# for-the-juan/SpGEMM

Hardware: AMD Instinct MI355X
Metric: SpGEMM GFLOPS (fp64, C=A^2) + achieved HBM GB/s fraction, 1/2/4/8 MI355X (higher is better)
Workload: dtype f64

## Files before the change

spgemm_amd/csrc/tsg_rows.hip:

```cpp
#include "tsg_internal.h"
#include "tsg_dev_common.h"

#include <cstdio>
#include <cstdlib>

namespace tsg {

namespace {

constexpr int S16_MAX = 16;
constexpr int RS_MAX = 64;
constexpr int CP_CH = 2048;
constexpr int S16_U = 2, S64_U = 2;
constexpr int M0_CAP = 256, M0_RUNS = 62, M0_NT = 64;
constexpr int M1_CAP = 512, M1_RUNS = 124, M1_NT = 128;
constexpr int M2_CAP = 1024, M2_RUNS = 248, M2_NT = 256;
constexpr int M3_CAP = 2048, M3_RUNS = 504, M3_NT = 512;
constexpr int M4_CAP = 4096, M4_RUNS = 512, M4_NT = 1024;
constexpr int W_CH = 32768;
constexpr int NCLS = 8;
constexpr int DR_SMAX = 4096;
constexpr int DR_CH = 16384;
constexpr int DR_GR = 16;
constexpr int DR_GMAX = 8192;
// ... 174 lines not shown
    if (P <= RS_MAX && k <= RS_MAX) return 1;
    if (P <= M0_CAP && k <= M0_RUNS) return 2;
    if (P <= M1_CAP && k <= M1_RUNS) return 3;
    if (P <= M2_CAP && k <= M2_RUNS) return 4;
    if (P <= M3_CAP && k <= M3_RUNS) return 5;
    if (P <= M4_CAP && k <= M4_RUNS) return 6;
    return 7;
}

__global__ __launch_bounds__(WG) void k_rows_bin(const int *rpA, int m, const long long *E, const long long *Etot,
                                                 int *rnnz, int4 *lists, int *cls, long long *soff,
                                                 unsigned long long *hst, const int *spart, int snb, int *sflag) {
    __shared__ int gb[NCLS];
    __shared__ long long red64[WAVES];
    constexpr int RPT = BIN_ROWS / WG;
    __shared__ int wcu[RPT][NCLS][WAVES];
    const int tid = threadIdx.x, lane = lane_id(), wv = wave_id();
    const int r0 = blockIdx.x * BIN_ROWS, r1 = min(m, r0 + BIN_ROWS);
    if (blockIdx.x == 0 && tid == 0) {
        hst[2] = (unsigned long long)*Etot;
        rnnz[m] = 0;
    }
    if (blockIdx.x == 0 && spart) {
        long long v = 0;
#pragma unroll 8
        for (int i = tid; i < snb; i += WG) v += spart[i];
        v = block_sum(v, red64);
        if (tid == 0 && v != 0) __hip_atomic_store(sflag, 1, __ATOMIC_RELAXED, __HIP_MEMORY_SCOPE_SYSTEM);
    }
    long long hp = 0, pmax = 0, drp = 0, hubr = 0, hbig = 0;
    int cu[RPT];
    int ra0[RPT], ra1[RPT];
#pragma unroll
    for (int u = 0; u < RPT; ++u) {
        const int r = r0 + u * WG + tid;
        ra0[u] = r < r1 ? rpA[r] : 0;
        ra1[u] = r < r1 ? rpA[r + 1] : 0;
    }
    long long e0[RPT], e1[RPT];
#pragma unroll
    for (int u = 0; u < RPT; ++u) {
        e0[u] = E[ra0[u]];
        e1[u] = E[ra1[u]];
    }
#pragma unroll
    for (int u = 0; u < RPT; ++u) {
        const int r = r0 + u * WG + tid;
        cu[u] = -1;
        if (r >= r1) continue;
        const long long P = e1[u] - e0[u];
        const int c = row_class(P, ra1[u] - ra0[u]);
        soff[r] = e0[u];
        cu[u] = c;
        if (c < 0) rnnz[r] = 0;
        hp += c == NCLS - 1 ? P : 0;
        hbig += c == NCLS - 1 && P <= kRowsHubProducts && P > OW_CH ? P - OW_CH : 0;
        pmax = max(pmax, P);
        if (P > kRowsHubProducts) drp += P;
        if (c == NCLS - 1 && ra1[u] - ra0[u] > OW_RUNS) ++hubr;
    }
    hp = block_sum(hp, red64);
    drp = block_sum(drp, red64);
    hubr = block_sum(hubr, red64);
    hbig = block_sum(hbig, red64);
#pragma unroll
    for (int d = 32; d > 0; d >>= 1) pmax = max(pmax, __shfl_xor(pmax, d, 64));
    if (lane == 0) red64[wv] = pmax;
    __syncthreads();
    if (tid == 0) {
        for (int w = 1; w < WAVES; ++w) pmax = max(pmax, red64[w]);
        if (hp) atomicAdd(&hst[0], (unsigned long long)hp);
        if (pmax) atomicMax(&hst[1], (unsigned long long)pmax);
        if (drp) atomicAdd(&hst[3], (unsigned long long)drp);
        if (hubr) atomicAdd(&hst[4], (unsigned long long)hubr);
        if (hbig) atomicAdd(&hst[8], (unsigned long long)hbig);
    }
    u64 mine[RPT];
#pragma unroll
    for (int u = 0; u < RPT; ++u) {
        mine[u] = 0;
#pragma unroll
        for (int t = 0; t < NCLS; ++t) {
            const u64 bt = __ballot(cu[u] == t);
            if (cu[u] == t) mine[u] = bt;
            if (lane == 0) wcu[u][t][wv] = __popcll(bt);
        }
    }
    __syncthreads();
    if (tid < NCLS) {
        int run = 0;
        for (int u = 0; u < RPT; ++u)
            for (int w = 0; w < WAVES; ++w) {
                const int v = wcu[u][tid][w];
                wcu[u][tid][w] = run;
                run += v;
            }
        gb[tid] = run ? atomicAdd(&cls[tid], run) : 0;
    }
    __syncthreads();
#pragma unroll
    for (int u = 0; u < RPT; ++u) {
        const int c = cu[u];
        if (c >= 0) {
            const int r = r0 + u * WG + tid;
            lists[(long)c * m + gb[c] + wcu[u][c][wv] + lanes_below(mine[u])] = make_int4(r, ra0[u], ra1[u] - ra0[u], 0);
        }
    }
}

constexpr int OH_NT = 1024, OH_PER = 8, OH_MAX = OH_NT * OH_PER, OH_NB = 64;
__global__ __launch_bounds__(OH_NT) void k_rows_order_h(const long long *E, const int *cls, int4 *list) {
    __shared__ int cnt[OH_NB];
    const int tid = threadIdx.x;
    const int n = cls[NCLS - 1];
    if (n < 2 || n > OH_MAX) return;
    if (tid < OH_NB) cnt[tid] = 0;
    __syncthreads();
    int4 r[OH_PER];
    int b[OH_PER];
#pragma unroll
    for (int u = 0; u < OH_PER; ++u) {
        const int i = u * OH_NT + tid;
        r[u] = i < n ? list[i] : make_int4(-1, 0, 0, 0);
    }
#pragma unroll
    for (int u = 0; u < OH_PER; ++u)
        if (r[u].x >= 0) {
            const long long P = E[r[u].y + r[u].z] - E[r[u].y];
            b[u] = OH_NB - 1 - (int)min((long long)OH_NB - 1, P >> 10);
            atomicAdd(&cnt[b[u]], 1);
        }
    __syncthreads();
    if (tid < 64) {
        const int v = cnt[tid];
        const int inc = wave_incl_scan_dpp(v);
        cnt[tid] = inc - v;
    }
    __syncthreads();
#pragma unroll
    for (int u = 0; u < OH_PER; ++u)
        if (r[u].x >= 0) list[atomicAdd(&cnt[b[u]], 1)] = r[u];
}

template <int J> __device__ __forceinline__ int row_bcast16(int v) {
    return __builtin_amdgcn_update_dpp(0, v, 0x150 | J, 0xf, 0xf, false);
}
template <int V> struct IntC { static constexpr int value = V; };
template <int J, int N, class F> __device__ __forceinline__ void static_for(F &&f) {
    if constexpr (J < N) {
        f(IntC<J>{});
        static_for<J + 1, N>(f);
    }
}

template <int G, int U>
__global__ __launch_bounds__(WG) void k_rows_small(RowsArgs g) {
    constexpr int RPW = 64 / G;
    __shared__ u64 sk[WAVES][U][64];
    __shared__ double sv[WAVES][U][64];
    const int lane = lane_id(), wv = wave_id(), sl = lane % G, gb = lane - sl;
    const int w0 = (blockIdx.x * WAVES + wv) * RPW * U;
    if (w0 >= g.nrows) return;
    int r[U], a0[U], k[U];
    bool live[U];
    long long base[U];
#pragma unroll
    for (int u = 0; u < U; ++u) {
        const int i = w0 + u * RPW + lane / G;
        live[u] = i < g.nrows;
        r[u] = 0, a0[u] = 0, k[u] = 0;
        if (live[u]) {
            const int4 e = g.list[i];
            r[u] = e.x;
            a0[u] = e.y;
            k[u] = e.z;
        }
    }
    int2 be[U];
    double av[U];
#pragma unroll
    for (int u = 0; u < U; ++u) {
        be[u] = make_int2(0, 0);
        av[u] = 0.0;
        base[u] = 0;
        if (live[u]) base[u] = g.E[a0[u]];
        if (sl < k[u]) {
            be[u] = g.ebnd[a0[u] + sl];
            av[u] = g.vA[a0[u] + sl];
        }
    }
    int P[U], pp[U];
    double ra[U];
#pragma unroll
    for (int u = 0; u < U; ++u) {
        const int len = be[u].y - be[u].x, bs = be[u].x;
        int inc = len;
        inc += dpp_mov<0x111, 0xf>(0, inc);
        inc += dpp_mov<0x112, 0xf>(0, inc);
        inc += dpp_mov<0x114, 0xf>(0, inc);
        inc += dpp_mov<0x118, 0xf>(0, inc);
        if constexpr (G == 64) {
            inc += dpp_mov<0x142, 0xa>(0, inc);
            inc += dpp_mov<0x143, 0xc>(0, inc);
        }
        const int roff = sl < k[u] ? inc - len : INT_MAX;
        int run = 0;
        if constexpr (G == 64) {
            P[u] = __shfl(inc, G - 1, G);
            for (int j = 1; j < k[u]; ++j) run = (__builtin_amdgcn_readlane(roff, j) <= sl) ? j : run;
        } else {
            static_assert(G == 16, "row broadcasts: 16-lane groups");
            P[u] = row_bcast16<15>(inc);
            static_for<1, 16>([&](auto jc) {
                constexpr int j = decltype(jc)::value;
                run = row_bcast16<j>(roff) <= sl ? j : run;
            });
        }
        const int rs = __shfl(roff, run, G), rb = __shfl(bs, run, G);
        ra[u] = __shfl(av[u], run, G);
        pp[u] = rb + sl - rs;
    }
    u64 key[U];
    double x[U];
#pragma unroll
    for (int u = 0; u < U; ++u) {
        key[u] = ~0ull;
        x[u] = 0.0;
        if (sl < P[u]) {
            key[u] = ((u64)(u32)g.Bcol[pp[u]] << 32) | (u32)sl;
            x[u] = g.Bval[pp[u]];
        }
    }
#pragma unroll
    for (int u = 0; u < U; ++u) {
        const u32 khi = (u32)(key[u] >> 32), klo = (u32)key[u];
        int rank = 0;
        if constexpr (G == 64) {
            for (int f = 0; f < P[u]; ++f) {
                const u64 kf = ((u64)(u32)__builtin_amdgcn_readlane((int)khi, f) << 32) |
                               (u32)__builtin_amdgcn_readlane((int)klo, f);
                rank += kf < key[u];
            }
        } else {
            const u64 ku = key[u];
            static_for<0, 16>([&](auto fc) {
                constexpr int f = decltype(fc)::value;
                const u64 kf = ((u64)(u32)row_bcast16<f>((int)khi) << 32) | (u32)row_bcast16<f>((int)klo);
                rank += kf < ku;
            });
        }
        if (sl < P[u]) {
            sk[wv][u][gb + rank] = key[u];
            sv[wv][u][gb + rank] = ra[u] * x[u];
        }
    }
    wave_lds_sync();
    const u64 gm = (G == 64 ? ~0ull : ((1ull << (G & 63)) - 1ull)) << gb;
#pragma unroll
    for (int u = 0; u < U; ++u) {
        int col = -1;
        bool head = false;
        if (sl < P[u]) {
            col = key_col(sk[wv][u][gb + sl]);
            head = sl == 0 || key_col(sk[wv][u][gb + sl - 1]) != col;
        }
        const u64 hb = __ballot(head) & gm;
        if (head) {
            double sm = sv[wv][u][gb + sl];
            for (int j = sl + 1; j < P[u] && key_col(sk[wv][u][gb + j]) == col; ++j) sm += sv[wv][u][gb + j];
            const long long o = base[u] + (long long)lanes_below(hb);
            g.Scol[o] = col;
            g.Sval[o] = sm;
        }
        if (live[u] && sl == 0) g.rnnz[r[u]] = __popcll(hb);
    }
}

template <int U, class T>
__device__ __forceinline__ void search_ilp(const T *a, int (&b)[U], int (&len)[U], const T (&key)[U],
                                           const bool (&ub)[U]) {
    for (;;) {
        bool more = false;
#pragma unroll
        for (int u = 0; u < U; ++u) more |= len[u] > 0;
        if (!more) break;
#pragma unroll
        for (int u = 0; u < U; ++u) {
            const int half = len[u] >> 1, idx = b[u] + half;
            const T v = a[len[u] > 0 ? idx : 0];
            const bool go = len[u] > 0 && (v < key[u] || (ub[u] && v == key[u]));
            b[u] = go ? idx + 1 : b[u];
            len[u] = go ? len[u] - half - 1 : half;
        }
    }
}

template <int D> __device__ __forceinline__ u32 lane_xor(u32 v) {
    if constexpr (D == 1) return (u32)__builtin_amdgcn_mov_dpp((int)v, 0xB1, 0xf, 0xf, false);
    else if constexpr (D == 2) return (u32)__builtin_amdgcn_mov_dpp((int)v, 0x4E, 0xf, 0xf, false);
    else if constexpr (D < 32) return (u32)__builtin_amdgcn_ds_swizzle((int)v, (D << 10) | 0x1f);
    else return (u32)__shfl_xor((int)v, D, 64);
}

template <int K, int J> __device__ __forceinline__ void bitonic_stage(u32 (&x)[4], int lane) {
    if constexpr (J >= 4) {
        constexpr int D = J / 4;
        const bool asc = K >= 256 || (lane & (K / 4)) == 0;
        const bool keep_max = asc != ((lane & D) == 0);
#pragma unroll
        for (int u = 0; u < 4; ++u) {
            const u32 y = lane_xor<D>(x[u]);
            x[u] = ((y < x[u]) != keep_max) ? y : x[u];
        }
    } else {
#pragma unroll
        for (int u = 0; u < 4; ++u)
            if ((u & J) == 0) {
                if constexpr (K < 4 || K >= 256) {
                    const bool asc = K < 4 ? (u & K) == 0 : true;
                    const u32 lo = min(x[u], x[u + J]), hi = max(x[u], x[u + J]);
                    x[u] = asc ? lo : hi;
                    x[u + J] = asc ? hi : lo;
                } else {
                    const bool desc = (lane & (K / 4)) != 0;
                    const bool sw = (x[u + J] < x[u]) != desc;
                    const u32 a = x[u], b = x[u + J];
                    x[u] = sw ? b : a;
                    x[u + J] = sw ? a : b;
                }
            }
    }
}
template <int K, int J> __device__ __forceinline__ void bitonic_merge(u32 (&x)[4], int lane) {
    bitonic_stage<K, J>(x, lane);
    if constexpr (J > 1) bitonic_merge<K, J / 2>(x, lane);
}
template <int K> __device__ __forceinline__ void bitonic_sort(u32 (&x)[4], int lane) {
    if constexpr (K > 2) bitonic_sort<K / 2>(x, lane);
    bitonic_merge<K, K / 2>(x, lane);
}
__device__ __forceinline__ void wave_sort256(u32 (&x)[4], int lane) { bitonic_sort<256>(x, lane); }

template <int NT, int CAP, int RUNS>
__global__ __launch_bounds__(NT, NT == 1024 ? 8 : 1) void k_rows_merge(RowsArgs g) {
    constexpr int NW = NT / 64;
    constexpr int IPM = (CAP + NT - 1) / NT | 1;
    constexpr int IB = CAP == 256 ? 8 : CAP == 512 ? 9 : CAP == 1024 ? 10 : CAP == 2048 ? 11 : 12;
    static_assert((1 << IB) == CAP, "CAP: a power of two in [256, 4096]");
    constexpr int SEG = 256;
    static_assert(CAP == 4 * NT, "four positions per thread");
    static_assert(RUNS <= NT, "a thread per A entry");
    __shared__ __align__(16) u32 kp[2][2][CAP];
    __shared__ int roff[RUNS + 1];
    __shared__ int rbs[RUNS];
    __shared__ double rav[RUNS];
    __shared__ int red[2 * NW];
    RP_INIT
    const int tid = threadIdx.x, lane = lane_id(), wv = wave_id();
    const int4 le = g.list[blockIdx.x];
    int2 be = make_int2(0, 0);
    double av = 0.0;
    if (tid < le.z) {
        be = g.ebnd[le.y + tid];
        av = g.vA[le.y + tid];
    }
    const long long base = g.E[le.y];
    double *const V = reinterpret_cast<double *>(kp[1][0]);
    {
        const int r = le.x;
        int k = 0, P = 0;
        {
            const int len = be.y - be.x;
            const u64 b = __ballot(len > 0);
            const int inc = wave_incl_scan_dpp(len);
            if (lane == 63) {
                red[wv] = __popcll(b);
                red[NW + wv] = inc;
            }
            __syncthreads();
            int off = 0, loff = 0;
#pragma unroll
            for (int w = 0; w < NW; ++w) {
                off += w < wv ? red[w] : 0;
                k += red[w];
                loff += w < wv ? red[NW + w] : 0;
                P += red[NW + w];
            }
            if (len > 0) {
                const int d = off + lanes_below(b);
                roff[d] = loff + inc - len;
                rbs[d] = be.x;
                rav[d] = av;
            }
            if (tid == 0) roff[k] = P;
            __syncthreads();
        }
        RP(0);
        const int e0 = wv * SEG + 4 * lane, ne = max(0, min(4, P - e0));
        int c[4] = {0, 0, 0, 0};
        u32 py[4] = {0, 0, 0, 0};
        double xv[4] = {0.0, 0.0, 0.0, 0.0};
        {
            int j = 0;
            if (ne > 0) j = lower_bound_dev(roff, 0, k + 1, e0 + 1) - 1;
            int pa[4] = {0, 0, 0, 0};
            double ra[4] = {0.0, 0.0, 0.0, 0.0}, bv[4] = {0.0, 0.0, 0.0, 0.0};
#pragma unroll
            for (int u = 0; u < 4; ++u)
                if (u < ne) {
                    const int q = e0 + u;
                    while (roff[j + 1] <= q) ++j;
                    pa[u] = rbs[j] + q - roff[j];
                    py[u] = ((u32)j << 16) | (u32)(q - roff[j]);
                    ra[u] = rav[j];
                }
#pragma unroll
            for (int u = 0; u < 4; ++u)
                if (u < ne) {
                    c[u] = g.Bcol[pa[u]];
                    bv[u] = g.Bval[pa[u]];
                }
#pragma unroll
            for (int u = 0; u < 4; ++u) xv[u] = u < ne ? ra[u] * bv[u] : 0.0;
        }
        int clo = INT_MAX, chi = -1;
#pragma unroll
        for (int u = 0; u < 4; ++u)
            if (u < ne) {
                clo = min(clo, c[u]);
                chi = max(chi, c[u]);
            }
        clo = wave_last(wave_incl_dpp(clo, INT_MAX, OpMin{}));
        chi = wave_last(wave_incl_dpp(chi, INT_MIN, OpMax{}));
        if (lane == 0) {
            red[wv] = clo;
            red[NW + wv] = chi;
        }
        __syncthreads();
        clo = red[0];
        chi = red[NW];
#pragma unroll
        for (int w = 1; w < NW; ++w) {
            clo = min(clo, red[w]);
            chi = max(chi, red[NW + w]);
        }
        const bool packed = (u32)(chi - clo) < (1u << (32 - IB)) - 1u;
        int npow = SEG;
        while (npow < P) npow <<= 1;
        u32 x[4] = {~0u, ~0u, ~0u, ~0u};
        if (packed) {
#pragma unroll
            for (int u = 0; u < 4; ++u) x[u] = u < ne ? ((u32)(c[u] - clo) << IB) | (u32)(e0 + u) : ~0u;
            if (ne > 0) {
                reinterpret_cast<double4 *>(V)[e0 >> 2] = make_double4(xv[0], xv[1], xv[2], xv[3]);
            }
            if (wv * SEG < P) wave_sort256(x, lane);
            if (wv * SEG < npow) *reinterpret_cast<uint4 *>(kp[0][0] + e0) = make_uint4(x[0], x[1], x[2], x[3]);
        } else {
#pragma unroll
            for (int u = 0; u < 4; ++u)
                if (u < ne) {
                    kp[0][0][e0 + u] = (u32)c[u];
                    kp[0][1][e0 + u] = py[u];
                }
        }
        __syncthreads();
        RP(1);
        int src = 0;
        if (packed) {
            const bool act = wv * SEG < npow;
            auto cmpx = [&](const uint4 y, bool rev, bool keep_min) {
                const u32 yy[4] = {rev ? y.w : y.x, rev ? y.z : y.y, rev ? y.y : y.z, rev ? y.x : y.w};
#pragma unroll
                for (int u = 0; u < 4; ++u) x[u] = keep_min ? min(x[u], yy[u]) : max(x[u], yy[u]);
            };
            for (int K = 2 * SEG; K <= npow; K <<= 1) {
                if (act) cmpx(*reinterpret_cast<const uint4 *>(kp[0][src] + (e0 ^ (K - 4))), true, (e0 & (K >> 1)) == 0);
                for (int J = K >> 2; J >= SEG; J >>= 1) {
                    src ^= 1;
                    if (act) *reinterpret_cast<uint4 *>(kp[0][src] + e0) = make_uint4(x[0], x[1], x[2], x[3]);
                    __syncthreads();
                    if (act) cmpx(*reinterpret_cast<const uint4 *>(kp[0][src] + (e0 ^ J)), false, (e0 & J) == 0);
                }
                if (act) bitonic_merge<256, 128>(x, lane);
                src ^= 1;
                if (act) *reinterpret_cast<uint4 *>(kp[0][src] + e0) = make_uint4(x[0], x[1], x[2], x[3]);
                __syncthreads();
            }
        }
        const int ipt = ((P + NT - 1) / NT) | 1;
        const int q0 = min(P, tid * ipt), q1 = min(P, q0 + ipt), nq = q1 - q0;
        if (!packed) {
            const int *const bd = roff;
            const int nb = k;
            int j0 = 0;
            if (nq > 0) j0 = lower_bound_dev(roff, 0, k + 1, q0 + 1) - 1;
            for (int lw = 0; (1 << lw) < nb; ++lw) {
                const u32 *ik = kp[src][0], *ip = kp[src][1];
                u32 *ok = kp[src ^ 1][0], *op = kp[src ^ 1][1];
                int pr = j0 >> (lw + 1);
                for (int q = q0; q < q1;) {
                    while (bd[min((pr + 1) << (lw + 1), nb)] <= q) ++pr;
                    const int ps = bd[pr << (lw + 1)];
                    const int pm = bd[min((2 * pr + 1) << lw, nb)];
                    const int pe = bd[min((pr + 1) << (lw + 1), nb)];
                    const int la = pm - ps, lb = pe - pm, qq = q - ps;
                    int lo = max(0, qq - lb), hi = min(qq, la);
                    while (lo < hi) {
                        const int t = (lo + hi) >> 1;
                        if (ik[ps + t] <= ik[pm + qq - t - 1]) lo = t + 1; else hi = t;
                    }
                    int ia = lo, ib = qq - lo;
                    u32 ka = ia < la ? ik[ps + ia] : ~0u, kbv = ib < lb ? ik[pm + ib] : ~0u;
                    const int qe = min(q1, pe);
                    for (; q < qe; ++q) {
                        const bool ta = ka <= kbv;
                        ok[q] = ta ? ka : kbv;
                        op[q] = ta ? ps + ia : pm + ib;
                        ia += ta;
                        ib += !ta;
                        const u32 kn = ik[ta ? ps + ia : pm + ib];
                        const bool live = ta ? ia < la : ib < lb;
                        ka = ta ? (live ? kn : ~0u) : ka;
                        kbv = ta ? kbv : (live ? kn : ~0u);
                    }
                }
#pragma unroll
                for (int u = 0; u < IPM; ++u)
                    if (u < nq) op[q0 + u] = ip[op[q0 + u]];
                __syncthreads();
                src ^= 1;
            }
        }
        RP(2);
        int nh = 0;
        const int np = packed ? max(0, min(4, P - e0)) : 0;
        double xs[4] = {0.0, 0.0, 0.0, 0.0};
        u32 hd = 0;
        const u32 *const sk = packed ? kp[0][src] : kp[src][0];
        double *const vb = reinterpret_cast<double *>(kp[src ^ 1][0]);
        if (packed) {
            const u32 prev = e0 > 0 && np > 0 ? sk[e0 - 1] : ~0u;
#pragma unroll
            for (int u = 0; u < 4; ++u)
                if (u < np) {
                    xs[u] = V[x[u] & (CAP - 1)];
                    const u32 pk = u ? x[u - 1] : prev;
                    hd |= (e0 + u == 0 || (x[u] >> IB) != (pk >> IB)) ? 1u << u : 0u;
                }
            nh = __popc(hd);
        } else {
            const u32 *sp = kp[src][1];
            int pa[IPM] = {};
            double ra[IPM] = {};
#pragma unroll
            for (int u = 0; u < IPM; ++u)
                if (u < nq) {
                    const u32 key = sk[q0 + u];
                    const u32 pj = sp[q0 + u];
                    const int ru = (int)(pj >> 16);
                    pa[u] = rbs[ru] + (int)(pj & 0xffffu);
                    ra[u] = rav[ru];
                    nh += (q0 + u == 0 || key != sk[q0 + u - 1]);
                }
            double xx[IPM] = {};
#pragma unroll
            for (int u = 0; u < IPM; ++u)
                if (u < nq) xx[u] = ra[u] * g.Bval[pa[u]];
#pragma unroll
            for (int u = 0; u < IPM; ++u)
                if (u < nq) vb[q0 + u] = xx[u];
        }
        const int inc = wave_incl_scan_dpp(nh);
        if (lane == 63) red[wv] = inc;
        __syncthreads();
        RP(3);
        int o = inc - nh, tot = 0;
#pragma unroll
        for (int w = 0; w < NW; ++w) {
            o += w < wv ? red[w] : 0;
            tot += red[w];
        }
        if (tid == 0) g.rnnz[r] = tot;
        if (packed) {
#pragma unroll
            for (int u = 0; u < 4; ++u)
                if (hd >> u & 1u) {
                    const u32 col = x[u] >> IB;
                    double sum = xs[u];
                    int j = u + 1;
#pragma unroll
                    for (int v = u + 1; v < 4; ++v)
                        if (j == v && v < np && (x[v] >> IB) == col) {
                            sum += xs[v];
                            ++j;
                        }
                    if (j == 4)
                        for (int q = e0 + 4; q < P && (sk[q] >> IB) == col; ++q) sum += V[sk[q] & (CAP - 1)];
                    g.Scol[base + o] = (int)col + clo;
                    g.Sval[base + o] = sum;
                    ++o;
                }
        } else {
            for (int q = q0; q < q1; ++q) {
                const u32 col = sk[q];
                if (q == 0 || sk[q - 1] != col) {
                    double sum = vb[q];
                    for (int j = q + 1; j < P && sk[j] == col; ++j) sum += vb[j];
                    g.Scol[base + o] = (int)col;
                    g.Sval[base + o] = sum;
                    ++o;
                }
            }
        }
        RP(4);
    }
    RP_DONE(CAP <= M1_CAP ? 2 : 1);
}

struct WalkTab {
    int pre[RH_NT];
    int bs[RH_NT];
    double av[RH_NT];
    int red[RH_NT / 64];
    int tot;
};
__device__ __forceinline__ void rows_batch(const RowsArgs &g, int a0, int k, int b0, WalkTab &tb) {
    constexpr int NW = RH_NT / 64;
    const int tid = threadIdx.x, lane = lane_id(), wv = wave_id();
    const int j = b0 + tid;
    int2 be = make_int2(0, 0);
    double av = 0.0;
    if (j < k) {
        be = g.ebnd[a0 + j];
        av = g.vA[a0 + j];
    }
    const int len = be.y - be.x;
    const int inc = wave_incl_scan_dpp(len);
    if (lane == 63) tb.red[wv] = inc;
    __syncthreads();
    int woff = 0, tot = 0;
#pragma unroll
    for (int w = 0; w < NW; ++w) {
        const int v = tb.red[w];
        woff += w < wv ? v : 0;
        tot += v;
    }
    tb.pre[tid] = woff + inc - len;
    tb.bs[tid] = be.x;
    tb.av[tid] = av;
    if (tid == 0) tb.tot = tot;
    __syncthreads();
}
__device__ __forceinline__ void batch_runmap(const WalkTab &tb, int nb, int qb, unsigned short *rmap, int *red) {
    constexpr int NW = RH_NT / 64;
    const int tid = threadIdx.x, lane = lane_id(), wv = wave_id();
    reinterpret_cast<uint2 *>(rmap)[tid] = make_uint2(0u, 0u);
    __syncthreads();
    if (tid < nb) {
        const int p0 = tb.pre[tid], p1 = tid + 1 < nb ? tb.pre[tid + 1] : tb.tot;
        if (p1 > p0 && p1 > qb && p0 < qb + 4 * RH_NT) rmap[max(p0, qb) - qb] = (unsigned short)tid;
    }
    __syncthreads();
    uint2 v = reinterpret_cast<const uint2 *>(rmap)[tid];
    int m[4];
    m[0] = (int)(v.x & 0xffffu);
    m[1] = max(m[0], (int)(v.x >> 16));
    m[2] = max(m[1], (int)(v.y & 0xffffu));
    m[3] = max(m[2], (int)(v.y >> 16));
    const int inc = wave_incl_dpp(m[3], 0, OpMax{});
    if (lane == 63) red[wv] = inc;
    int carry = __shfl_up(inc, 1, 64);
    if (lane == 0) carry = 0;
    __syncthreads();
#pragma unroll
    for (int w = 0; w < NW; ++w) carry = w < wv ? max(carry, red[w]) : carry;
    v.x = (u32)max(m[0], carry) | ((u32)max(m[1], carry) << 16);
    v.y = (u32)max(m[2], carry) | ((u32)max(m[3], carry) << 16);
    reinterpret_cast<uint2 *>(rmap)[tid] = v;
    __syncthreads();
}

template <bool VAL, class F>
__device__ __forceinline__ void batch_walk(const RowsArgs &g, int nb, int q0, int q1, const WalkTab &tb, F &&f,
                                           unsigned short *rmap, int *red) {
    constexpr int U = 4;
    const int tid = threadIdx.x;
    if (q0 >= q1) return;
    int c[U], cn[U];
    double x[U], xn[U];
    auto fetch = [&](int qb, unsigned short *rm, int (&cc)[U], double (&xx)[U]) {
        __syncthreads();
        batch_runmap(tb, nb, qb, rm, red);
#pragma unroll
        for (int u = 0; u < U; ++u) {
            const int q = qb + u * RH_NT + tid;
            const int r = q < q1 ? rm[u * RH_NT + tid] : 0;
            const int bs = tb.bs[r], pre = tb.pre[r];
            const int pp = q < q1 ? bs + q - pre : 0;
            cc[u] = g.Bcol[pp];
            if (VAL) xx[u] = g.Bval[pp];
        }
    };
    auto use = [&](int qb, const unsigned short *rm, const int (&cc)[U], const double (&xx)[U]) {
#pragma unroll
        for (int u = 0; u < U; ++u) {
            const bool ok = qb + u * RH_NT + tid < q1;
            f(cc[u], VAL && ok ? tb.av[rm[u * RH_NT + tid]] * xx[u] : 0.0, ok);
        }
    };
    constexpr int STEP = U * RH_NT;
    unsigned short *const rm0 = rmap, *const rm1 = rmap + 4 * RH_NT;
    fetch(q0, rm0, c, x);
#pragma unroll
    for (int st = 0; st < W_CH / STEP; st += 2) {
        const int qb = q0 + st * STEP;
        if (qb >= q1) break;
        fetch(qb + STEP, rm1, cn, xn);
        use(qb, rm0, c, x);
        if (qb + STEP >= q1) break;
        fetch(qb + 2 * STEP, rm0, c, x);
        use(qb + STEP, rm1, cn, xn);
    }
}

__device__ __forceinline__ int bm_rank(const u64 *bm, const u16 *g4, const int *blk, long long c) {
    const int w = (int)(c >> 6), gi = w >> 2, sub = w & 3;
    const ulonglong2 lo = reinterpret_cast<const ulonglong2 *>(bm)[gi * 2];
    const ulonglong2 hi = reinterpret_cast<const ulonglong2 *>(bm)[gi * 2 + 1];
    const u64 word = sub == 0 ? lo.x : sub == 1 ? lo.y : sub == 2 ? hi.x : hi.y;
    int rk = blk[w / RH_BLK] + g4[gi] + __popcll(word & ((1ull << (c & 63)) - 1ull));
    rk += sub > 0 ? __popcll(lo.x) : 0;
    rk += sub > 1 ? __popcll(lo.y) : 0;
    rk += sub > 2 ? __popcll(hi.x) : 0;
    return rk;
}

__global__ __launch_bounds__(RH_NT) void k_rows_bitmap(RowsArgs g, int *Tc, double *Tx, int *Tr,
                                                      unsigned long long *tcur) {
    {
        const int4 le0 = g.list[blockIdx.x];
        if (g.E[le0.y + le0.z] - g.E[le0.y] > kRowsHubProducts) return;
    }
    __shared__ __align__(16) u64 bm[RH_WORDS];
    __shared__ u16 g4[RH_NGRP];
    __shared__ int blk[RH_NBLK];
    __shared__ WalkTab wt;
    __shared__ int red[3 * (RH_NT / 64)];
    constexpr int NW = RH_NT / 64;
    RP_INIT
    const int tid = threadIdx.x, lane = lane_id(), wv = wave_id();
    const int4 le = g.list[blockIdx.x];
    const int r = le.x, a0 = le.y, k = le.z;
    const long long base = g.E[a0];
    if (k > OW_RUNS) return;
    const int P = (int)(g.E[a0 + k] - base);
    int *const opre = reinterpret_cast<int *>(&wt);
    int *const obs = opre + OW_RUNS;
    int lo = INT_MAX, hi = -1;
    {
        int2 be0 = make_int2(0, 0), be1 = make_int2(0, 0);
        if (2 * tid < k) be0 = g.ebnd[a0 + 2 * tid];
        if (2 * tid + 1 < k) be1 = g.ebnd[a0 + 2 * tid + 1];
        const int l0 = be0.y - be0.x, l1 = be1.y - be1.x;
        const int f0 = l0 > 0 ? g.Bcol[be0.x] : INT_MAX, e0 = l0 > 0 ? g.Bcol[be0.y - 1] : -1;
        const int f1 = l1 > 0 ? g.Bcol[be1.x] : INT_MAX, e1 = l1 > 0 ? g.Bcol[be1.y - 1] : -1;
        const int inc = wave_incl_scan_dpp(l0 + l1);
        lo = wave_last(wave_incl_dpp(min(f0, f1), INT_MAX, OpMin{}));
        hi = wave_last(wave_incl_dpp(max(e0, e1), INT_MIN, OpMax{}));
        if (lane == 63) red[wv] = inc;
        if (lane == 0) {
            red[NW + wv] = lo;
            red[2 * NW + wv] = hi;
        }
        __syncthreads();
        int woff = 0;
#pragma unroll
        for (int w = 0; w < NW; ++w) {
            woff += w < wv ? red[w] : 0;
            lo = min(lo, red[NW + w]);
            hi = max(hi, red[2 * NW + w]);
        }
        const int ex = woff + inc - l0 - l1;
        opre[2 * tid] = ex;
        opre[2 * tid + 1] = ex + l0;
        obs[2 * tid] = be0.x;
        obs[2 * tid + 1] = be1.x;
    }
    if ((long long)hi - lo >= RH_SPAN) return;
    {
        __shared__ long long s_toff;
        if (tid == 0 && P > OW_CH) s_toff = (long long)atomicAdd(tcur, (unsigned long long)(P - OW_CH));
// ... 400 lines not shown
    for (int t = 0; t < PT; ++t) {
        const int w = tid * PT + t;
        v[t] = w < nw ? in[u0 + w] : 0;
        sum += v[t];
    }
    const int inc = wave_incl_scan_dpp(sum);
    if (lane == 63) red[wv] = inc;
    __syncthreads();
    int off = inc - sum, tot = 0;
#pragma unroll
    for (int w = 0; w < NW; ++w) {
        off += w < wv ? red[w] : 0;
        tot += red[w];
    }
    long long rb = 0;
    int lo = 0, wb = 0, row = 0;
    if (rec) {
        const int4 le = g.list[blockIdx.x];
        rb = g.E[le.y];
        row = le.x;
        lo = wlo[blockIdx.x];
        wb = wwb[blockIdx.x];
    }
#pragma unroll
    for (int t = 0; t < PT; ++t) {
        const int w = tid * PT + t;
        if (w < nw) {
            out[u0 + w] = off;
            if (rec) rec[u0 + w] = WUnit{rb + off, lo + (w << wb), wb, v[t], row};
        }
        off += v[t];
    }
    if (rnnz && tid == 0) rnnz[g.list[blockIdx.x].x] = tot;
    if (ulist) {
        constexpr int HEAVY = W_RPT * WU_NT;
        int ns = 0, nh = 0, nm = 0;
#pragma unroll
        for (int t = 0; t < PT; ++t) {
            ns += v[t] > 0 && v[t] <= WS_MAX;
            nh += v[t] > HEAVY;
            nm += v[t] > WS_MAX && v[t] <= HEAVY;
        }
        const int is = wave_incl_scan_dpp(ns), ih = wave_incl_scan_dpp(nh), im = wave_incl_scan_dpp(nm);
        unsigned long long old = 0;
        if (lane == 63 && (is | ih | im))
            old = atomicAdd(lcnt64, (unsigned long long)is | ((unsigned long long)ih << 21) |
                                        ((unsigned long long)im << 42));
        old = ((unsigned long long)__shfl((int)(old >> 32), 63, 64) << 32) | (u32)__shfl((int)old, 63, 64);
        int ps = (int)(old & 0x1fffff) + is - ns, ph = (int)((old >> 21) & 0x1fffff) + ih - nh,
            pm = (int)(old >> 42) + im - nm;
#pragma unroll
        for (int t = 0; t < PT; ++t) {
            const int w = tid * PT + t;
            if (v[t] > 0 && v[t] <= WS_MAX) ulist[ps++] = u0 + w;
            else if (v[t] > HEAVY) ulist2[nu - 1 - ph++] = u0 + w;
            else if (v[t] > WS_MAX) ulist2[pm++] = u0 + w;
        }
    }
}

__global__ __launch_bounds__(W_NT) __attribute__((amdgpu_waves_per_eu(8, 8))) void k_rows_wscatter(RowsArgs g, const int4 *chunks, const long long *cmoff,
                                                       const int *wlo, const int *wwb, const int *ubase,
                                                       const int *ubo, const int *cbo) {
    __shared__ __align__(16) unsigned char lds[W_MAXW * 4 + 8 * RH_NT * 2];
    __shared__ WalkTab wt;
    __shared__ int red[W_NT / 64];
    int *const cur = reinterpret_cast<int *>(lds);
    unsigned short *const rm = reinterpret_cast<unsigned short *>(lds + W_MAXW * 4);
    const int tid = threadIdx.x;
    const int4 ch = chunks[blockIdx.x];
    const int u0 = ubase[ch.x], nw = ubase[ch.x + 1] - u0;
    const int lo = wlo[ch.x], wb = wwb[ch.x];
    const int *const cb = cbo + cmoff[blockIdx.x];
    for (int w = tid; w < nw; w += W_NT) cur[w] = ubo[u0 + w] + cb[w];
    const int4 le = g.list[ch.x];
    const int a0 = le.y, k = le.z, b0 = ch.y * RH_NT;
    rows_batch(g, a0, k, b0, wt);
    const long long base = g.E[a0];
    const int q0 = ch.z * W_CH, q1 = min(wt.tot, q0 + W_CH), nb = min(RH_NT, k - b0);
    batch_walk<true>(g, nb, q0, q1, wt, [&](int c, double x, bool v) {
        const int lane = lane_id();
        const int w = v ? (c - lo) >> wb : -1;
        int len;
        const u64 bm = wave_runs(w, &len);
        int b = 0;
        if (v && (bm >> lane & 1ull)) b = atomicAdd(&cur[w], len);
        const int hl = 63 - __builtin_clzll(bm & ((2ull << lane) - 1ull));
        const int hb = __shfl(b, hl, 64);
        if (v) {
            const long long o = base + hb + (lane - hl);
            g.Scol[o] = c;
            g.Sval[o] = x;
        }
    }, rm, red);
}

__device__ __forceinline__ int w_rank(const u64 *bm, const u16 *g4, const int *blk, int c) {
    const int w = c >> 6, gi = w >> 2, sub = w & 3;
    const ulonglong2 lo = reinterpret_cast<const ulonglong2 *>(bm)[gi * 2];
    const ulonglong2 hi = reinterpret_cast<const ulonglong2 *>(bm)[gi * 2 + 1];
    const u64 word = sub == 0 ? lo.x : sub == 1 ? lo.y : sub == 2 ? hi.x : hi.y;
    int rk = blk[w / W_BLK] + g4[gi] + __popcll(word & ((1ull << (c & 63)) - 1ull));
    rk += sub > 0 ? __popcll(lo.x) : 0;
    rk += sub > 1 ? __popcll(lo.y) : 0;
    rk += sub > 2 ? __popcll(hi.x) : 0;
    return rk;
}

template <int MODE, int NT>
__global__ __launch_bounds__(NT) void k_rows_wunit(RowsArgs g, const WUnit *urec, int *ucount, const int *uoff,
                                                    const int *Crp, int *Ccol, double *Cval,
                                                    const int *ulist = nullptr, int ulast = 0,
                                                    int nheavy = 0) {
    constexpr int NW = NT / 64;
    __shared__ __align__(16) u64 bm[W_WORDS];
    __shared__ u16 g4[W_WORDS / 4];
    __shared__ int blk[W_NBLK];
    __shared__ __align__(16) double vals[W_VCAP];
    __shared__ int red[NW];
    RP_INIT
    const int tid = threadIdx.x, lane = lane_id(), wv = wave_id();
    const int b = blockIdx.x;
    const int u = ulist ? ulist[b < nheavy ? ulast - b : b - nheavy] : b;
    const WUnit R = urec[u];
    const int n = R.n;
    if (n == 0) {
        if (MODE == 0 && tid == 0) ucount[u] = 0;
        return;
    }
    const int wb = R.wb;
    const long long wlo0 = R.wlo0;
    const long long s0 = R.s0;
    const int nwd = 1 << (wb - 6);
    if constexpr (MODE == 0) {
        for (int w = tid; w < nwd; w += NT) bm[w] = 0ull;
        int cc[W_RPT];
#pragma unroll
        for (int t = 0; t < W_RPT; ++t) {
            const int q = t * NT + tid;
            cc[t] = q < n ? (int)(g.Scol[s0 + q] - wlo0) : -1;
        }
        __syncthreads();
#pragma unroll
        for (int t = 0; t < W_RPT; ++t)
            if (cc[t] >= 0) atomicOr(&bm[cc[t] >> 6], 1ull << (cc[t] & 63));
        for (int q = W_RPT * NT + tid; q < n; q += NT) {
            const int c = (int)(g.Scol[s0 + q] - wlo0);
            atomicOr(&bm[c >> 6], 1ull << (c & 63));
        }
        __syncthreads();
        int cnt = 0;
        for (int w = tid; w < nwd; w += NT) cnt += __popcll(bm[w]);
        cnt = wave_sum(cnt);
        if (lane == 0) red[wv] = cnt;
        __syncthreads();
        if (tid == 0) {
            int t = 0;
#pragma unroll
            for (int w = 0; w < NW; ++w) t += red[w];
            ucount[u] = t;
        }
        RP_DONE(0);
        return;
    }
    for (int w = tid; w < nwd; w += NT) bm[w] = 0ull;
    int cc[W_RPT];
    double xx[W_RPT];
#pragma unroll
    for (int t = 0; t < W_RPT; ++t) {
        const int q = t * NT + tid;
        cc[t] = q < n ? (int)(g.Scol[s0 + q] - wlo0) : -1;
        xx[t] = q < n ? g.Sval[s0 + q] : 0.0;
    }
    const long long o0 = (long long)Crp[R.row] + uoff[u];
    __syncthreads();
#pragma unroll
    for (int t = 0; t < W_RPT; ++t)
        if (cc[t] >= 0) atomicOr(&bm[cc[t] >> 6], 1ull << (cc[t] & 63));
    for (int q = W_RPT * NT + tid; q < n; q += NT) {
        const int c = (int)(g.Scol[s0 + q] - wlo0);
        atomicOr(&bm[c >> 6], 1ull << (c & 63));
    }
    __syncthreads();
    RP(1);
    for (int bb = wv; bb * W_BLK < nwd; bb += NW) {
        const int w0 = bb * W_BLK + lane * 8;
        int t0 = 0, t1 = 0;
#pragma unroll
        for (int v = 0; v < 4; ++v) {
            t0 += w0 + v < nwd ? __popcll(bm[w0 + v]) : 0;
            t1 += w0 + 4 + v < nwd ? __popcll(bm[w0 + 4 + v]) : 0;
        }
        const int inc = wave_incl_scan_dpp(t0 + t1);
        if (w0 < nwd) g4[w0 / 4] = (u16)(inc - t0 - t1);
        if (w0 + 4 < nwd) g4[w0 / 4 + 1] = (u16)(inc - t1);
        if (lane == 63) blk[bb] = inc;
    }
    __syncthreads();
    const int nb = (nwd + W_BLK - 1) / W_BLK;
    if (wv == 0) {
        const int v = lane < nb ? blk[lane] : 0;
        const int inc = wave_incl_scan_dpp(v);
        if (lane < nb) blk[lane] = inc - v;
        if (lane == 63) red[0] = inc;
    }
    __syncthreads();
    const int wn = red[0];
    RP(2);
    int rk[W_RPT];
#pragma unroll
    for (int t = 0; t < W_RPT; ++t) rk[t] = cc[t] >= 0 ? w_rank(bm, g4, blk, cc[t]) : 0;
    static_assert(2 * W_WORDS >= W_RPT * NT, "the bitmap's LDS holds a column per rank (wn <= n)");
    if (n <= W_RPT * NT) {
        int *const cl = reinterpret_cast<int *>(bm);
        __syncthreads();
#pragma unroll
        for (int t = 0; t < W_RPT; ++t)
            if (cc[t] >= 0) cl[rk[t]] = cc[t];
        RP(3);
        for (int r0 = 0; r0 < wn; r0 += W_VCAP) {
            const int r1 = min(wn, r0 + W_VCAP);
            for (int j = tid; j < r1 - r0; j += NT) vals[j] = 0.0;
            __syncthreads();
#pragma unroll
            for (int t = 0; t < W_RPT; ++t)
                if (cc[t] >= 0 && (unsigned)(rk[t] - r0) < (unsigned)W_VCAP) atomicAdd(&vals[rk[t] - r0], xx[t]);
            __syncthreads();
            RP(4);
            for (int j = tid; j < r1 - r0; j += NT) {
                Ccol[o0 + r0 + j] = (int)(wlo0 + cl[r0 + j]);
                Cval[o0 + r0 + j] = vals[j];
            }
            __syncthreads();
            RP(5);
        }
        RP_DONE(0);
        return;
    }
#ifdef TSG_ROWS_PROF
    for (int k = 0; k < 3; ++k) {
        rp_acc[6 + k] += rp_acc[k];
        rp_acc[k] = 0;
    }
#endif
    for (int r0 = 0; r0 < wn; r0 += W_VCAP) {
        const int r1 = min(wn, r0 + W_VCAP);
        for (int j = tid; j < r1 - r0; j += NT) vals[j] = 0.0;
        __syncthreads();
#pragma unroll
        for (int t = 0; t < W_RPT; ++t)
            if (cc[t] >= 0 && (unsigned)(rk[t] - r0) < (unsigned)W_VCAP) atomicAdd(&vals[rk[t] - r0], xx[t]);
        for (int q = W_RPT * NT + tid; q < n; q += NT) {
            const int c = (int)(g.Scol[s0 + q] - wlo0);
            const int rq = w_rank(bm, g4, blk, c) - r0;
            if ((unsigned)rq < (unsigned)W_VCAP) atomicAdd(&vals[rq], g.Sval[s0 + q]);
        }
        __syncthreads();
        RP(9);
        for (int w = tid; w < nwd; w += NT) {
            u64 word = bm[w];
            if (!word) continue;
            int r = w_rank(bm, g4, blk, w * 64);
            if (r >= r1) continue;
            while (word) {
                const int bit = __builtin_ctzll(word);
                word &= word - 1ull;
                if (r >= r0 && r < r1) {
                    Ccol[o0 + r] = (int)(wlo0 + w * 64 + bit);
                    Cval[o0 + r] = vals[r - r0];
                }
                ++r;
            }
        }
        __syncthreads();
        RP(10);
    }
    RP(11);
    RP_DONE(0);
}

__global__ __launch_bounds__(WS_NT) void k_rows_wsort(RowsArgs g, const WUnit *urec, const int *ulist,
                                                    const int *uoff, const int *Crp, int *Ccol, double *Cval) {
    constexpr int NW = WS_NT / 64, SEG = 256, IB = WS_CAP == 1024 ? 10 : WS_CAP == 2048 ? 11 : 12;
    static_assert((1 << IB) == WS_CAP && (W_WBMAX + IB) < 32, "keys: window column and position in a u32");
    __shared__ __align__(16) u32 kb[2][WS_CAP];
    __shared__ __align__(16) double V[WS_CAP];
    __shared__ int red[NW];
    const int u = ulist[blockIdx.x];
    const WUnit R = urec[u];
    const int n = R.n;
    const int tid = threadIdx.x, lane = lane_id(), wv = wave_id();
    const int e0 = 4 * tid;
    u32 x[4];
    double xv[4];
#pragma unroll
    for (int k = 0; k < 4; ++k) {
        const int q = e0 + k;
        x[k] = q < n ? ((u32)(g.Scol[R.s0 + q] - R.wlo0) << IB) | (u32)q : ~0u;
        xv[k] = q < n ? g.Sval[R.s0 + q] : 0.0;
    }
    const long long o0 = (long long)Crp[R.row] + uoff[u];
    int npow = SEG;
    while (npow < n) npow <<= 1;
    const bool act = wv * SEG < npow;
    if (e0 < n) reinterpret_cast<double4 *>(V)[tid] = make_double4(xv[0], xv[1], xv[2], xv[3]);
    if (wv * SEG < n) wave_sort256(x, lane);
    if (act) *reinterpret_cast<uint4 *>(kb[0] + e0) = make_uint4(x[0], x[1], x[2], x[3]);
    __syncthreads();
    int src = 0;
    auto cmpx = [&](const uint4 y, bool rev, bool keep_min) {
        const u32 yy[4] = {rev ? y.w : y.x, rev ? y.z : y.y, rev ? y.y : y.z, rev ? y.x : y.w};
#pragma unroll
        for (int k = 0; k < 4; ++k) x[k] = keep_min ? min(x[k], yy[k]) : max(x[k], yy[k]);
    };
    for (int K = 2 * SEG; K <= npow; K <<= 1) {
        if (act) cmpx(*reinterpret_cast<const uint4 *>(kb[src] + (e0 ^ (K - 4))), true, (e0 & (K >> 1)) == 0);
        for (int J = K >> 2; J >= SEG; J >>= 1) {
            src ^= 1;
            if (act) *reinterpret_cast<uint4 *>(kb[src] + e0) = make_uint4(x[0], x[1], x[2], x[3]);
            __syncthreads();
            if (act) cmpx(*reinterpret_cast<const uint4 *>(kb[src] + (e0 ^ J)), false, (e0 & J) == 0);
        }
        if (act) bitonic_merge<256, 128>(x, lane);
        src ^= 1;
        if (act) *reinterpret_cast<uint4 *>(kb[src] + e0) = make_uint4(x[0], x[1], x[2], x[3]);
        __syncthreads();
    }
    const u32 *const ks = kb[src];
    u32 prev = e0 > 0 && e0 - 1 < n ? ks[e0 - 1] >> IB : ~0u;
    bool hd[4];
    int nh = 0;
#pragma unroll
    for (int k = 0; k < 4; ++k) {
        const u32 col = x[k] >> IB;
        hd[k] = e0 + k < n && col != prev;
        prev = col;
        nh += hd[k];
    }
    const int inc = wave_incl_scan_dpp(nh);
    if (lane == 63) red[wv] = inc;
    __syncthreads();
    int rk = inc - nh;
#pragma unroll
    for (int w = 0; w < NW; ++w) rk += w < wv ? red[w] : 0;
#pragma unroll
    for (int k = 0; k < 4; ++k)
        if (hd[k]) {
            const u32 col = x[k] >> IB;
            double sum = V[x[k] & (WS_CAP - 1)];
            for (int p = e0 + k + 1; p < n; ++p) {
                const u32 y = ks[p];
                if ((y >> IB) != col) break;
                sum += V[y & (WS_CAP - 1)];
            }
            Ccol[o0 + rk] = (int)(R.wlo0 + (long long)col);
            Cval[o0 + rk] = sum;
            ++rk;
        }
}

struct DrRow {
    long long base;
    int r, bs, L, nu;
    double aL;
};
struct DrEnt {
    int p;
    int nd;
    int col;
    int dup;
    double val;
};
constexpr int DR_NT = 1024;

__global__ __launch_bounds__(DR_NT) void k_rows_dr_prep(RowsArgs g, long long *soff, DrRow *rows, DrEnt *ents,
                                                        int *ord, int4 *chunks, int *nchunk, int *ndr,
                                                        int enq) {
    constexpr int NW = DR_NT / 64;
    __shared__ unsigned long long sk[DR_SMAX];
    __shared__ double sv[DR_SMAX];
    __shared__ int red[2 * NW + 2];
    const int tid = threadIdx.x, lane = lane_id(), wv = wave_id();
    const int4 le = g.list[blockIdx.x];
    const int r = le.x, a0 = le.y, k = le.z;
    const long long base = g.E[a0];
    const long long P = g.E[a0 + k] - base;
    if (P <= kRowsHubProducts) return;
    int jl;
    const long long L = row_longest_run(g.E, a0, k, &jl, red);
    const int nS = (int)(P - L);
    if (nS > DR_SMAX) return;
    __shared__ int s_h;
    if (tid == 0) s_h = atomicAdd(ndr, 1);
    const long long eL = g.E[a0 + jl] - base;
    const int2 bL = g.ebnd[a0 + jl];
    int npow = 1;
    while (npow < nS) npow <<= 1;
    for (int q = tid; q < npow; q += DR_NT) {
        if (q >= nS) {
            sk[q] = ~0ull;
            continue;
        }
        const long long qq = base + (q < eL ? q : q + L);
        int lo = a0, hi = a0 + k;
        while (hi - lo > 1) {
            const int mid = (lo + hi) >> 1;
            if (g.E[mid] <= qq) lo = mid; else hi = mid;
        }
        const int pb = g.ebnd[lo].x + (int)(qq - g.E[lo]);
        const int c = g.Bcol[pb];
        sv[q] = g.vA[lo] * g.Bval[pb];
        sk[q] = ((unsigned long long)(unsigned)c << 12) | (unsigned)q;
    }
    __syncthreads();
    for (int K = 2; K <= npow; K <<= 1)
        for (int J = K >> 1; J > 0; J >>= 1) {
            for (int i = tid; i < npow; i += DR_NT) {
                const int ij = i ^ J;
                if (ij > i) {
                    const unsigned long long a = sk[i], b = sk[ij];
                    const bool asc = (i & K) == 0;
                    if ((a > b) == asc) {
                        sk[i] = b;
                        sk[ij] = a;
                    }
                }
            }
            __syncthreads();
        }
    int nh = 0;
    int hq[DR_SMAX / DR_NT];
#pragma unroll
    for (int u = 0; u < DR_SMAX / DR_NT; ++u) {
        const int t = tid * (DR_SMAX / DR_NT) + u;
        hq[u] = t < nS && (t == 0 || (sk[t] >> 12) != (sk[t - 1] >> 12));
        nh += hq[u];
    }
    const int inc = wave_incl_scan_dpp(nh);
    if (lane == 63) red[wv] = inc;
    __syncthreads();
    int o = inc - nh, nu = 0;
#pragma unroll
    for (int w = 0; w < NW; ++w) {
        o += w < wv ? red[w] : 0;
        nu += red[w];
    }
    const int h = s_h;
    DrEnt *const E8 = ents + (long)h * DR_SMAX;
    const int oslot = o;
    int ndp = 0;
    int mydup[DR_SMAX / DR_NT];
#pragma unroll
    for (int u = 0; u < DR_SMAX / DR_NT; ++u) {
        const int t = tid * (DR_SMAX / DR_NT) + u;
        mydup[u] = 0;
        if (!hq[u]) continue;
        const int c = (int)(sk[t] >> 12);
        double sum = sv[sk[t] & 4095u];
        for (int j = t + 1; j < nS && (int)(sk[j] >> 12) == c; ++j) sum += sv[sk[j] & 4095u];
        int lo = 0, hi = (int)L;
        while (lo < hi) {
            const int mid = (lo + hi) >> 1;
            if (g.Bcol[bL.x + mid] < c) lo = mid + 1; else hi = mid;
        }
        mydup[u] = lo < L && g.Bcol[bL.x + lo] == c;
        ndp += !mydup[u];
        DrEnt e;
        e.p = lo;
        e.col = c;
        e.dup = mydup[u];
        e.val = sum;
        e.nd = 0;
        E8[o++] = e;
    }
    __syncthreads();
    const int inc2 = wave_incl_scan_dpp(ndp);
    if (lane == 63) red[wv] = inc2;
    __syncthreads();
    int nd = inc2 - ndp, ndt = 0;
#pragma unroll
    for (int w = 0; w < NW; ++w) {
        nd += w < wv ? red[w] : 0;
        ndt += red[w];
    }
    int os = oslot;
#pragma unroll
    for (int u = 0; u < DR_SMAX / DR_NT; ++u) {
        if (!hq[u]) continue;
        E8[os].nd = nd;
        nd += !mydup[u];
        ++os;
    }
    if (tid == 0) {
        DrRow d;
        d.base = base;
        d.r = r;
        d.bs = bL.x;
        d.L = (int)L;
        d.nu = nu;
        d.aL = g.vA[a0 + jl];
        rows[h] = d;
        g.rnnz[r] = (int)L + ndt;
        soff[r] = -1;
        if (enq) {
            ord[h] = h;
            const int nch = (int)((L + DR_CH - 1) / DR_CH);
            const int c0 = atomicAdd(nchunk, nch);
            for (int c = 0; c < nch; ++c) chunks[c0 + c] = make_int4(h, 1, c * DR_CH, 0);
        }
    }
}

__global__ __launch_bounds__(DR_NT) void k_rows_dr_group(const DrRow *rows, const int *ndrp, int *ord, int4 *chunks,
                                                         int *nchunk) {
    constexpr int NW = DR_NT / 64, PT = DR_GMAX / DR_NT;
    __shared__ unsigned long long sk[DR_GMAX];
    __shared__ int red[NW];
    const int tid = threadIdx.x, lane = lane_id(), wv = wave_id();
    const int n = *ndrp;
    int npow = 1;
    while (npow < n) npow <<= 1;
    for (int q = tid; q < npow; q += DR_NT)
        sk[q] = q < n ? ((unsigned long long)(unsigned)rows[q].bs << 32) | (unsigned)q : ~0ull;
    __syncthreads();
    for (int K = 2; K <= npow; K <<= 1)
        for (int J = K >> 1; J > 0; J >>= 1) {
            for (int i = tid; i < npow; i += DR_NT) {
                const int ij = i ^ J;
                if (ij > i) {
                    const unsigned long long a = sk[i], b = sk[ij];
                    const bool asc = (i & K) == 0;
                    if ((a > b) == asc) {
                        sk[i] = b;
                        sk[ij] = a;
                    }
                }
            }
            __syncthreads();
        }
    int cnt[PT], tot = 0;
#pragma unroll
    for (int u = 0; u < PT; ++u) {
        const int i = tid * PT + u;
        cnt[u] = 0;
        if (i >= n) continue;
        const unsigned run = (unsigned)(sk[i] >> 32);
        int lo = 0, hi = i;
        while (lo < hi) {
            const int mid = (lo + hi) >> 1;
            if ((unsigned)(sk[mid] >> 32) < run) lo = mid + 1; else hi = mid;
        }
        if ((i - lo) % DR_GR == 0) cnt[u] = (rows[(unsigned)sk[i]].L + DR_CH - 1) / DR_CH;
        tot += cnt[u];
    }
    const int inc = wave_incl_scan_dpp(tot);
    if (lane == 63) red[wv] = inc;
    __syncthreads();
    int o = inc - tot, all = 0;
#pragma unroll
    for (int w = 0; w < NW; ++w) {
        o += w < wv ? red[w] : 0;
        all += red[w];
    }
#pragma unroll
    for (int u = 0; u < PT; ++u) {
        const int i = tid * PT + u;
        if (i < n) ord[i] = (int)(unsigned)sk[i];
        if (!cnt[u]) continue;
        const unsigned run = (unsigned)(sk[i] >> 32);
        int lo = 0, hi = i;
        while (lo < hi) {
            const int mid = (lo + hi) >> 1;
            if ((unsigned)(sk[mid] >> 32) < run) lo = mid + 1; else hi = mid;
        }
        int e = i + 1, eh = n;
        while (e < eh) {
            const int mid = (e + eh) >> 1;
            if ((unsigned)(sk[mid] >> 32) <= run) e = mid + 1; else eh = mid;
        }
        const int R = cnt[u], S = (e - lo + DR_GR - 1) / DR_GR, sb = (i - lo) / DR_GR;
        const int gbase = o - sb * R;
        const int nr = min(DR_GR, e - i);
        for (int c = 0; c < R; ++c) chunks[gbase + c * S + sb] = make_int4(i, nr, c * DR_CH, 0);
        o += R;
    }
    if (tid == 0) *nchunk = all;
}

constexpr int DR_FU = DR_CH / DR_NT;
__global__ __launch_bounds__(DR_NT) void k_rows_dr_fill(RowsArgs g, const int *Crp, int *Ccol, double *Cval,
                                                        const DrRow *rows, const DrEnt *ents, const int *ord,
                                                        const int4 *chunks, const int *nchunk) {
    __shared__ int sp[DR_SMAX];
    __shared__ int snd[DR_SMAX];
    __shared__ unsigned char sdup[DR_SMAX];
    __shared__ double sval[DR_SMAX];
    __shared__ int r_lo[DR_GR], r_hi[DR_GR], r_nd0[DR_GR], r_h[DR_GR], r_out[DR_GR];
    __shared__ double r_a[DR_GR];
    const int tid = threadIdx.x;
    const int nck = *nchunk;
    for (int q = blockIdx.x; q < nck; q += gridDim.x) {
        const int4 ch = chunks[q];
        const int nr = ch.y, i0 = ch.z;
        const DrRow d0 = rows[ord[ch.x]];
        const int i1 = min(d0.L, i0 + DR_CH);
        const bool last = i1 == d0.L;
        int c[DR_FU];
        double v[DR_FU];
#pragma unroll
        for (int u = 0; u < DR_FU; ++u) {
            const int i = i0 + u * DR_NT + tid;
            c[u] = i < i1 ? g.Bcol[d0.bs + i] : 0;
            v[u] = i < i1 ? g.Bval[d0.bs + i] : 0.0;
        }
        if (tid < 2 * nr) {
            const int j = tid >> 1, hi_side = tid & 1;
            const int h = ord[ch.x + j];
            const DrRow d = rows[h];
            const DrEnt *const E8 = ents + (long)h * DR_SMAX;
            const int key = hi_side ? (last ? d.L + 1 : i1) : i0;
            int lo = 0, hi = d.nu;
            while (lo < hi) {
                const int mid = (lo + hi) >> 1;
                if (E8[mid].p < key) lo = mid + 1; else hi = mid;
            }
            if (hi_side) {
                r_hi[j] = lo;
            } else {
                r_lo[j] = lo;
                r_h[j] = h;
// ... 578 lines not shown
```

Baseline: 113.2.

## Branchless bitonic compare-exchange and skip dead segments in bitonic sorts

Result: faster. 123.0, median of 6 (+8.6%).

```diff
diff --git a/spgemm_amd/csrc/tsg_rows.hip b/spgemm_amd/csrc/tsg_rows.hip
--- a/spgemm_amd/csrc/tsg_rows.hip
+++ b/spgemm_amd/csrc/tsg_rows.hip
@@ -500,16 +500,18 @@
     else return (u32)__shfl_xor((int)v, D, 64);
 }
 
+__device__ __forceinline__ u32 minmax_sel(u32 a, u32 b, u32 sel) { return min(max(a, b), max(min(a, b), sel)); }
+template <int B> __device__ __forceinline__ u32 bit_fill(u32 v) { return (u32)((int)(v << (31 - B)) >> 31); }
+constexpr int ilog2_c(int v) { return v <= 1 ? 0 : 1 + ilog2_c(v >> 1); }
+
 template <int K, int J> __device__ __forceinline__ void bitonic_stage(u32 (&x)[4], int lane) {
     if constexpr (J >= 4) {
         constexpr int D = J / 4;
-        const bool asc = K >= 256 || (lane & (K / 4)) == 0;
-        const bool keep_max = asc != ((lane & D) == 0);
-#pragma unroll
-        for (int u = 0; u < 4; ++u) {
-            const u32 y = lane_xor<D>(x[u]);
-            x[u] = ((y < x[u]) != keep_max) ? y : x[u];
-        }
+        u32 w = (u32)lane;
+        if constexpr (K < 256) w ^= bit_fill<ilog2_c(K / 4)>((u32)lane);
+        const u32 sel = bit_fill<ilog2_c(D)>(w);
+#pragma unroll
+        for (int u = 0; u < 4; ++u) x[u] = minmax_sel(x[u], lane_xor<D>(x[u]), sel);
     } else {
 #pragma unroll
         for (int u = 0; u < 4; ++u)
@@ -520,11 +522,10 @@
                     x[u] = asc ? lo : hi;
                     x[u + J] = asc ? hi : lo;
                 } else {
-                    const bool desc = (lane & (K / 4)) != 0;
-                    const bool sw = (x[u + J] < x[u]) != desc;
+                    const u32 desc = bit_fill<ilog2_c(K / 4)>((u32)lane);
                     const u32 a = x[u], b = x[u + J];
-                    x[u] = sw ? b : a;
-                    x[u + J] = sw ? a : b;
+                    x[u] = minmax_sel(a, b, desc);
+                    x[u + J] = minmax_sel(a, b, ~desc);
                 }
             }
     }
@@ -537,7 +538,44 @@
     if constexpr (K > 2) bitonic_sort<K / 2>(x, lane);
     bitonic_merge<K, K / 2>(x, lane);
 }
-__device__ __forceinline__ void wave_sort256(u32 (&x)[4], int lane) { bitonic_sort<256>(x, lane); }
+__device__ __forceinline__ void wave_sort256(u32 (&x)[4], int lane, int live) {
+    bitonic_sort<64>(x, lane);
+    if (live > 64) bitonic_merge<128, 64>(x, lane);
+    if (live > 128) bitonic_merge<256, 128>(x, lane);
+}
+
+template <int STRIDE>
+__device__ __forceinline__ int xwave_merge(u32 (&x)[4], u32 *kb, int lane, int wv, int P, int npow) {
+    constexpr int SEG = 256;
+    wv = __builtin_amdgcn_readfirstlane(wv);
+    npow = __builtin_amdgcn_readfirstlane(npow);
+    const int nlive = (__builtin_amdgcn_readfirstlane(P) + SEG - 1) / SEG;
+    const bool live = wv < nlive;
+    const int e0 = wv * SEG + 4 * lane;
+    int src = 0;
+    auto cmpx = [&](int pw, int off, bool rev) {
+        if (pw >= nlive) return;
+        const uint4 y = *reinterpret_cast<const uint4 *>(kb + src * STRIDE + off);
+        const u32 yy[4] = {rev ? y.w : y.x, rev ? y.z : y.y, rev ? y.y : y.z, rev ? y.x : y.w};
+        const u32 sel = pw < wv ? ~0u : 0u;
+#pragma unroll
+        for (int u = 0; u < 4; ++u) x[u] = minmax_sel(x[u], yy[u], sel);
+    };
+    for (int K = 2 * SEG; K <= npow; K <<= 1) {
+        if (live) cmpx(wv ^ (K / SEG - 1), e0 ^ (K - 4), true);
+        for (int J = K >> 2; J >= SEG; J >>= 1) {
+            src ^= 1;
+            if (live) *reinterpret_cast<uint4 *>(kb + src * STRIDE + e0) = make_uint4(x[0], x[1], x[2], x[3]);
+            __syncthreads();
+            if (live) cmpx(wv ^ (J / SEG), e0 ^ J, false);
+        }
+        if (live) bitonic_merge<256, 128>(x, lane);
+        src ^= 1;
+        if (live) *reinterpret_cast<uint4 *>(kb + src * STRIDE + e0) = make_uint4(x[0], x[1], x[2], x[3]);
+        __syncthreads();
+    }
+    return src;
+}
 
 template <int NT, int CAP, int RUNS>
 __global__ __launch_bounds__(NT, NT == 1024 ? 8 : 1) void k_rows_merge(RowsArgs g) {
@@ -652,8 +690,11 @@
             if (ne > 0) {
                 reinterpret_cast<double4 *>(V)[e0 >> 2] = make_double4(xv[0], xv[1], xv[2], xv[3]);
             }
-            if (wv * SEG < P) wave_sort256(x, lane);
-            if (wv * SEG < npow) *reinterpret_cast<uint4 *>(kp[0][0] + e0) = make_uint4(x[0], x[1], x[2], x[3]);
+            const int live = __builtin_amdgcn_readfirstlane(P - wv * SEG);
+            if (live > 0) {
+                wave_sort256(x, lane, live);
+                *reinterpret_cast<uint4 *>(kp[0][0] + e0) = make_uint4(x[0], x[1], x[2], x[3]);
+            }
         } else {
 #pragma unroll
             for (int u = 0; u < 4; ++u)
@@ -665,27 +706,7 @@
         __syncthreads();
         RP(1);
         int src = 0;
-        if (packed) {
-            const bool act = wv * SEG < npow;
-            auto cmpx = [&](const uint4 y, bool rev, bool keep_min) {
-                const u32 yy[4] = {rev ? y.w : y.x, rev ? y.z : y.y, rev ? y.y : y.z, rev ? y.x : y.w};
-#pragma unroll
-                for (int u = 0; u < 4; ++u) x[u] = keep_min ? min(x[u], yy[u]) : max(x[u], yy[u]);
-            };
-            for (int K = 2 * SEG; K <= npow; K <<= 1) {
-                if (act) cmpx(*reinterpret_cast<const uint4 *>(kp[0][src] + (e0 ^ (K - 4))), true, (e0 & (K >> 1)) == 0);
-                for (int J = K >> 2; J >= SEG; J >>= 1) {
-                    src ^= 1;
-                    if (act) *reinterpret_cast<uint4 *>(kp[0][src] + e0) = make_uint4(x[0], x[1], x[2], x[3]);
-                    __syncthreads();
-                    if (act) cmpx(*reinterpret_cast<const uint4 *>(kp[0][src] + (e0 ^ J)), false, (e0 & J) == 0);
-                }
-                if (act) bitonic_merge<256, 128>(x, lane);
-                src ^= 1;
-                if (act) *reinterpret_cast<uint4 *>(kp[0][src] + e0) = make_uint4(x[0], x[1], x[2], x[3]);
-                __syncthreads();
-            }
-        }
+        if (packed) src = xwave_merge<CAP>(x, kp[0][0], lane, wv, P, npow);
         const int ipt = ((P + NT - 1) / NT) | 1;
         const int q0 = min(P, tid * ipt), q1 = min(P, q0 + ipt), nq = q1 - q0;
         if (!packed) {
@@ -1692,30 +1713,14 @@
     const long long o0 = (long long)Crp[R.row] + uoff[u];
     int npow = SEG;
     while (npow < n) npow <<= 1;
-    const bool act = wv * SEG < npow;
     if (e0 < n) reinterpret_cast<double4 *>(V)[tid] = make_double4(xv[0], xv[1], xv[2], xv[3]);
-    if (wv * SEG < n) wave_sort256(x, lane);
-    if (act) *reinterpret_cast<uint4 *>(kb[0] + e0) = make_uint4(x[0], x[1], x[2], x[3]);
-    __syncthreads();
-    int src = 0;
-    auto cmpx = [&](const uint4 y, bool rev, bool keep_min) {
-        const u32 yy[4] = {rev ? y.w : y.x, rev ? y.z : y.y, rev ? y.y : y.z, rev ? y.x : y.w};
-#pragma unroll
-        for (int k = 0; k < 4; ++k) x[k] = keep_min ? min(x[k], yy[k]) : max(x[k], yy[k]);
-    };
-    for (int K = 2 * SEG; K <= npow; K <<= 1) {
-        if (act) cmpx(*reinterpret_cast<const uint4 *>(kb[src] + (e0 ^ (K - 4))), true, (e0 & (K >> 1)) == 0);
-        for (int J = K >> 2; J >= SEG; J >>= 1) {
-            src ^= 1;
-            if (act) *reinterpret_cast<uint4 *>(kb[src] + e0) = make_uint4(x[0], x[1], x[2], x[3]);
-            __syncthreads();
-            if (act) cmpx(*reinterpret_cast<const uint4 *>(kb[src] + (e0 ^ J)), false, (e0 & J) == 0);
-        }
-        if (act) bitonic_merge<256, 128>(x, lane);
-        src ^= 1;
-        if (act) *reinterpret_cast<uint4 *>(kb[src] + e0) = make_uint4(x[0], x[1], x[2], x[3]);
-        __syncthreads();
-    }
+    const int live = __builtin_amdgcn_readfirstlane(n - wv * SEG);
+    if (live > 0) {
+        wave_sort256(x, lane, live);
+        *reinterpret_cast<uint4 *>(kb[0] + e0) = make_uint4(x[0], x[1], x[2], x[3]);
+    }
+    __syncthreads();
+    const int src = xwave_merge<WS_CAP>(x, kb[0], lane, wv, n, npow);
     const u32 *const ks = kb[src];
     u32 prev = e0 > 0 && e0 - 1 < n ? ks[e0 - 1] >> IB : ~0u;
     bool hd[4];
```
